# zyc-123/InstanceDiff

Hardware: AMD Instinct MI355X
Metric: denoising steps/sec (256x256 bs16) (higher is better)
Workload: dtype f32; 1 GPU; 256x256 1-ch synthetic, 1000-step reverse chain, batch 16 per GPU, 2 UNet fwd + reverse update per step; global_batch=16, parallelism=replicas x1 (no collective)

## Files before the change

instancediff_amd/csrc/conv_wino4.hip:

```cpp
#include <stdlib.h>

#include <type_traits>

#include "conv_args.h"

using idiff_detail::ConvArgs;

namespace {

constexpr int CK = 4;
constexpr int TW = 32, TH = 16;
constexpr int RCOLS = TW + 2;
constexpr int RS = 40;
constexpr int TRH = TH + 2;
constexpr int PS = TRH * RS;
constexpr int PSP = 768;
constexpr int NT = 512;
constexpr int NL = 6;
constexpr int R_FLOATS = NL * NT;
constexpr int V_FLOATS = 9 * 2 * 64 * 4;
constexpr int U_FLOATS = 9 * 4 * 64 * 4;

typedef float floatx2 __attribute__((ext_vector_type(2)));

__host__ __device__ constexpr int PF(int u) { return (3 * u + 1) / 2; }
__host__ __device__ constexpr int PH(int u) { return 1 + 3 * (u / 2); }
__host__ __device__ constexpr int pos(int u, int v) { return v < 4 ? 4 * PF(u) + v : 4 * PH(u) + 2 * (u & 1) + (v - 4); }

struct Geo4 {
    int np;
    int total;
    int tiles_y8;
};

template <int CTRL>
__device__ __forceinline__ float dpp_row_shr(float v) {
    return __builtin_bit_cast(float, __builtin_amdgcn_update_dpp(0, __builtin_bit_cast(int, v), CTRL, 0xf, 0xf, true));
}
__device__ __forceinline__ float row_sum16(float v) {
    v += dpp_row_shr<0x111>(v);
    v += dpp_row_shr<0x112>(v);
    v += dpp_row_shr<0x114>(v);
    v += dpp_row_shr<0x118>(v);
    return v;
}

#ifdef IDIFF_WINO_TRACE
#define TRACE_PARAM , long long* trace
#define TRACE_INIT long long tr_t[9] = {0, 0, 0, 0, 0, 0, 0, 0, 0}, tr_acc[8] = {0, 0, 0, 0, 0, 0, 0, 0};
#define TRACE_MARK(k)                                                  \
    tr_t[k] = __builtin_readcyclecounter();                            \
    if (k > 0) tr_acc[k - 1] += tr_t[k] - tr_t[k - 1];                 \
    else if (tr_t[3] != 0) tr_acc[3] += tr_t[0] - tr_t[3];
#define TRACE_FINI                                                                                                      \
    if (tid == 0) {                                                                                                     \
        for (int q_ = 0; q_ < 8; ++q_) atomicAdd((unsigned long long*)trace + q_, (unsigned long long)tr_acc[q_]);      \
    }
#else
#define TRACE_PARAM
#define TRACE_INIT
#define TRACE_MARK(k)
#define TRACE_FINI
#endif
#ifdef IDIFF_WINO_SLOTS
#define SLOT_INIT long long sl_acc[10] = {0, 0, 0, 0, 0, 0, 0, 0, 0, 0}, sl_t = 0;
#define SLOT_START sl_t = __builtin_readcyclecounter();
#define SLOT_MARK(k)                                        \
    {                                                       \
        const long long t_ = __builtin_readcyclecounter();  \
        sl_acc[k] += t_ - sl_t;                             \
        sl_t = t_;                                          \
    }
#define SLOT_FINI                                                                                                                   \
    if (lane == 0) {                                                                                                                \
        long long w_ = 0;                                                                                                           \
        for (int q_ = 0; q_ < 9; ++q_) w_ += sl_acc[q_];                                                                            \
        atomicAdd((unsigned long long*)trace + 8 + 2 * wave, (unsigned long long)w_);                                               \
        atomicAdd((unsigned long long*)trace + 9 + 2 * wave, (unsigned long long)sl_acc[9]);                                        \
    }
#else
#define SLOT_INIT
#define SLOT_START
#define SLOT_MARK(k)
#define SLOT_FINI
#endif

__device__ __forceinline__ const float* scalar_ptr(const float* p) {
    const unsigned long long v = reinterpret_cast<unsigned long long>(p);
    const unsigned lo = __builtin_amdgcn_readfirstlane((unsigned)v), hi = __builtin_amdgcn_readfirstlane((unsigned)(v >> 32));
    return reinterpret_cast<const float*>(((unsigned long long)hi << 32) | lo);
}

__device__ __forceinline__ void bt6(const float (&x)[6], float (&o)[6]) {
    o[0] = __builtin_fmaf(4.f, x[0], __builtin_fmaf(-5.f, x[2], x[4]));
    const float p = __builtin_fmaf(-4.f, x[2], x[4]), q = __builtin_fmaf(-4.f, x[1], x[3]);
    o[1] = p + q;
    o[2] = p - q;
    const float c = x[4] - x[2], e = x[3] - x[1];
    o[3] = __builtin_fmaf(2.f, e, c);
    o[4] = __builtin_fmaf(-2.f, e, c);
    o[5] = __builtin_fmaf(4.f, x[1], __builtin_fmaf(-5.f, x[3], x[5]));
}
__device__ __forceinline__ void at6(const float x0, const float x1, const float x2, const float x3, const float x4, const float x5, float (&o)[4]) {
    const float s1 = x1 + x2, d1 = x1 - x2, s2 = x3 + x4, d2 = x3 - x4;
    o[0] = (x0 + s1) + s2;
    o[1] = __builtin_fmaf(2.f, d2, d1);
    o[2] = __builtin_fmaf(4.f, s2, s1);
    o[3] = __builtin_fmaf(8.f, d2, d1) + x5;
}

template <int MODE, int SPEC, bool RAG, bool HEAVY>
__device__ __forceinline__ void conv_wino4_body(const ConvArgs& a, const Geo4& g, float* smem TRACE_PARAM) {
    float* const Rb = smem;
    float* const Vb = smem + 3 * R_FLOATS;
    float* const Ub = Vb + 2 * V_FLOATS;
    float* const econst = Ub + 2 * U_FLOATS;
    int* const gtab = reinterpret_cast<int*>(econst + 512);
    constexpr unsigned R_BYTES = R_FLOATS * 4, U_BYTES = U_FLOATS * 4;
    const unsigned lds_base = __builtin_amdgcn_readfirstlane((unsigned)reinterpret_cast<unsigned long long>(smem));
    const unsigned U_LDS0 = lds_base + (3 * R_FLOATS + 2 * V_FLOATS) * 4;

    const int tid = threadIdx.x;
    const int lane = tid & 63;
    const int wave = __builtin_amdgcn_readfirstlane(tid >> 6);
    const int k4 = lane >> 4;
    const int cb = wave & 3;
    const int tblk = wave >> 2;
    const int HWin = a.Hin * a.Win;
    const int nchunks = a.Cin / CK;

    constexpr int RSRC_FLAGS = 0x00020000;
    struct View {
        int b, co0, y0, x0;
    };
    const float *p0A = a.src0, *p1A = a.src0, *puA = a.wwino4, *p0B = a.src0, *p1B = a.src0, *puB = a.wwino4;
    View vA = {0, 0, 0, 0}, vB = {0, 0, 0, 0};
    int nrB = 0;
    unsigned omaskA = 0, omaskB = 0;
    int it_b = 0, it_cob = 0, it_px = 0, it_py = 0;
    const int tiles_y = g.np / a.tiles_x;
    int d_cob, d_px, d_py, d_b;
    {
        const int G0 = gridDim.x;
        d_cob = G0 % a.ncob;
        const int r1 = G0 / a.ncob;
        d_px = r1 % a.tiles_x;
        const int r2 = r1 / a.tiles_x;
        d_py = r2 % tiles_y;
        d_b = r2 / tiles_y;
    }
    auto decode_first = [&](int item) {
        it_cob = item % a.ncob;
        const int r1 = item / a.ncob;
        it_px = r1 % a.tiles_x;
        const int r2 = r1 / a.tiles_x;
        it_py = r2 % tiles_y;
        it_b = r2 / tiles_y;
    };
    auto advance_item = [&]() {
        it_cob += d_cob;
        int carry = it_cob >= a.ncob;
        it_cob -= carry ? a.ncob : 0;
        it_px += d_px + carry;
        carry = it_px >= a.tiles_x;
        it_px -= carry ? a.tiles_x : 0;
        it_py += d_py + carry;
        carry = it_py >= tiles_y;
        it_py -= carry ? tiles_y : 0;
        it_b += d_b + carry;
    };
    auto decode_B = [&]() {
        vB.b = it_b, vB.co0 = it_cob * 64, vB.y0 = it_py * TH, vB.x0 = it_px * TW;
        puB = scalar_ptr(a.wwino4 + (long long)it_cob * U_FLOATS);
        p0B = scalar_ptr(a.src0 + (long long)it_b * a.bs0);
        p1B = scalar_ptr(SPEC == 3 ? a.src1 + (long long)it_b * a.bs1 : a.src0);
        nrB = 0x7fffffff;
    };
    auto write_table = [&](const View& v) {
        int t = tid;
        asm volatile("" : "+v"(t));
        unsigned om = 0;
#pragma unroll
        for (int i = 0; i < NL; ++i) {
            const int e = t + i * NT;
            const int ci = e / PSP;
            const int rem = e - ci * PSP;
            const int r = rem / RS;
            const int c = rem - r * RS;
            const int oy = v.y0 - 1 + r, ox = v.x0 - 1 + c;
            const bool in = rem < PS && c < RCOLS && (unsigned)oy < (unsigned)a.Hout && (unsigned)ox < (unsigned)a.Wout;
            const int sp = MODE == IDIFF_CONV_UPSAMPLE2 ? (oy >> 1) * a.Win + (ox >> 1) : oy * a.Win + ox;
            gtab[i * NT + tid] = in ? (ci * HWin + sp) * 4 : -1;
            om |= (in ? 0u : 1u) << i;
        }
        return om;
    };
    auto shift_B_to_A = [&]() { p0A = p0B, p1A = p1B, puA = puB, vA = vB, omaskA = omaskB; };
    const int ustride_b = a.ncob * U_FLOATS * 4;

    typedef const __attribute__((address_space(4))) floatx4* cfloatx4p;
    struct Pro {
        floatx4 a, b;
    };
    auto load_pro = [&](int p) {
        Pro r;
        if (SPEC == 2) {
            const bool inA = p < nchunks;
            const long long o = (long long)(inA ? vA.b : vB.b) * a.C0r + (inA ? p : p - nchunks) * CK;
            r.a = *(cfloatx4p)(a.pro_a + o);
            r.b = *(cfloatx4p)(a.pro_b + o);
        }
        return r;
    };

    const unsigned u_voff = tid * 16;
    auto dma_u = [&](int p, int buf) {
        const bool inA = p < nchunks;
        const int so = (inA ? p : p - nchunks) * ustride_b;
        const __amdgpu_buffer_rsrc_t rsu = __builtin_amdgcn_make_buffer_rsrc(const_cast<float*>(inA ? puA : puB), 0, inA ? 0x7fffffff : nrB, RSRC_FLAGS);
        const unsigned lds0 = __builtin_amdgcn_readfirstlane(U_LDS0 + (unsigned)buf * U_BYTES + (unsigned)wave * 1024u);
        asm volatile(
            "s_nop 4\n\ts_mov_b32 m0, %2\n\ts_nop 0\n\tbuffer_load_dwordx4 %0, %1, %3 offen lds\n\t"
            "s_add_u32 m0, m0, 0x2000\n\ts_nop 0\n\tbuffer_load_dwordx4 %0, %1, %4 offen lds\n\t"
            "s_add_u32 m0, m0, 0x2000\n\ts_nop 0\n\tbuffer_load_dwordx4 %0, %1, %5 offen lds\n\t"
            "s_add_u32 m0, m0, 0x2000\n\ts_nop 0\n\tbuffer_load_dwordx4 %0, %1, %6 offen lds"
            ::"v"(u_voff), "s"(rsu), "s"(lds0), "s"(so), "s"(so + NT * 16), "s"(so + 2 * NT * 16), "s"(so + 3 * NT * 16)
            : "memory", "scc");
        if (!HEAVY) {
            const unsigned lds4 = __builtin_amdgcn_readfirstlane(lds0 + 4 * NT * 16 - 256 * 16);
            asm volatile("s_nop 4\n\ts_mov_b32 m0, %2\n\ts_nop 0\n\tbuffer_load_dwordx4 %0, %1, %3 offen lds" ::"v"(u_voff), "s"(rsu), "s"(lds4),
                         "s"(so + 4 * NT * 16 - 256 * 16)
                         : "memory");
        }
    };
    auto dma_u_piece = [&](int p, int buf, int i) {
        const bool inA = p < nchunks;
        const int so = (inA ? p : p - nchunks) * ustride_b + (i < 4 ? i * NT * 16 : 4 * NT * 16 - 256 * 16);
        const __amdgpu_buffer_rsrc_t rsu = __builtin_amdgcn_make_buffer_rsrc(const_cast<float*>(inA ? puA : puB), 0, inA ? 0x7fffffff : nrB, RSRC_FLAGS);
        const unsigned lds0 = __builtin_amdgcn_readfirstlane(U_LDS0 + (unsigned)buf * U_BYTES + (unsigned)wave * 1024u + (unsigned)(i < 4 ? i * NT * 16 : 4 * NT * 16 - 256 * 16));
        asm volatile("s_nop 4\n\ts_mov_b32 m0, %2\n\ts_nop 0\n\tbuffer_load_dwordx4 %0, %1, %3 offen lds" ::"v"(u_voff), "s"(rsu), "s"(lds0), "s"(so) : "memory");
    };
    auto dma_raw = [&](int p, unsigned rslot) {
        const bool inA = p < nchunks;
        const int cbase = (inA ? p : p - nchunks) * CK;
        int goff[NL];
#pragma unroll
        for (int i = 0; i < NL; ++i) goff[i] = gtab[i * NT + tid];
        const int C0v = a.C0v;
        const bool second = SPEC == 3 && cbase >= C0v;
        const unsigned long long b0 = reinterpret_cast<unsigned long long>(inA ? p0A : p0B), b1 = reinterpret_cast<unsigned long long>(inA ? p1A : p1B);
        const float* const base = reinterpret_cast<const float*>(second ? b1 : b0);
        const int so = (second ? cbase - C0v : cbase) * HWin * 4;
        const __amdgpu_buffer_rsrc_t rs = __builtin_amdgcn_make_buffer_rsrc(const_cast<float*>(base), 0, inA ? 0x7fffffff : nrB, RSRC_FLAGS);
        const unsigned lds0 = __builtin_amdgcn_readfirstlane(lds_base + rslot + (unsigned)wave * 256u);
        asm volatile(
            "s_nop 4\n\ts_mov_b32 m0, %8\n\ts_nop 0\n\tbuffer_load_dword %0, %6, %7 offen lds\n\t"
            "s_add_u32 m0, m0, 0x800\n\ts_nop 0\n\tbuffer_load_dword %1, %6, %7 offen lds\n\t"
            "s_add_u32 m0, m0, 0x800\n\ts_nop 0\n\tbuffer_load_dword %2, %6, %7 offen lds\n\t"
            "s_add_u32 m0, m0, 0x800\n\ts_nop 0\n\tbuffer_load_dword %3, %6, %7 offen lds\n\t"
            "s_add_u32 m0, m0, 0x800\n\ts_nop 0\n\tbuffer_load_dword %4, %6, %7 offen lds\n\t"
            "s_add_u32 m0, m0, 0x800\n\ts_nop 0\n\tbuffer_load_dword %5, %6, %7 offen lds"
            ::"v"(goff[0]), "v"(goff[1]), "v"(goff[2]), "v"(goff[3]), "v"(goff[4]), "v"(goff[5]), "s"(rs), "s"(so), "s"(lds0)
            : "memory", "scc");
    };
    auto dma_raw_piece = [&](int p, unsigned rslot, int i, int goff_i) {
        const bool inA = p < nchunks;
        const int cbase = (inA ? p : p - nchunks) * CK;
        const int C0v = a.C0v;
        const bool second = SPEC == 3 && cbase >= C0v;
        const unsigned long long b0 = reinterpret_cast<unsigned long long>(inA ? p0A : p0B), b1 = reinterpret_cast<unsigned long long>(inA ? p1A : p1B);
        const float* const base = reinterpret_cast<const float*>(second ? b1 : b0);
        const int so = (second ? cbase - C0v : cbase) * HWin * 4;
        const __amdgpu_buffer_rsrc_t rs = __builtin_amdgcn_make_buffer_rsrc(const_cast<float*>(base), 0, inA ? 0x7fffffff : nrB, RSRC_FLAGS);
        const unsigned lds0 = __builtin_amdgcn_readfirstlane(lds_base + rslot + (unsigned)wave * 256u + (unsigned)i * 2048u);
        asm volatile("s_nop 4\n\ts_mov_b32 m0, %3\n\ts_nop 0\n\tbuffer_load_dword %0, %1, %2 offen lds" ::"v"(goff_i), "s"(rs), "s"(so), "s"(lds0) : "memory");
    };
    float rinA[NL], rinB[NL];
    auto ld_raw = [&](float (&dst)[NL], int p, int i, int goff_i) {
        const bool inA = p < nchunks;
        const int so = (inA ? p : p - nchunks) * CK * HWin * 4;
        const __amdgpu_buffer_rsrc_t rs = __builtin_amdgcn_make_buffer_rsrc(const_cast<float*>(inA ? p0A : p0B), 0, inA ? 0x7fffffff : nrB, RSRC_FLAGS);
        asm volatile("s_nop 4\n\tbuffer_load_dword %0, %1, %2, %3 offen" : "=v"(dst[i]) : "v"(goff_i), "s"(rs), "s"(so) : "memory");
    };
    auto stage_act = [&](const float (&src)[NL], int p, const Pro& pro, unsigned rslot, int i0, int i1) {
        const unsigned om = p < nchunks ? omaskA : omaskB;
        float* const R = reinterpret_cast<float*>(reinterpret_cast<char*>(Rb) + rslot) + tid;
        constexpr bool hiw = !HEAVY;
#pragma unroll
        for (int i = 0; i < NL; ++i) {
            if (i < i0 || i >= i1) continue;
            const float pa = i == 0 ? pro.a.x : i == 1 ? (hiw ? pro.a.y : pro.a.x) : i == 2 ? pro.a.y : i == 3 ? pro.a.z : i == 4 ? (hiw ? pro.a.w : pro.a.z) : pro.a.w;
            const float pb = i == 0 ? pro.b.x : i == 1 ? (hiw ? pro.b.y : pro.b.x) : i == 2 ? pro.b.y : i == 3 ? pro.b.z : i == 4 ? (hiw ? pro.b.w : pro.b.z) : pro.b.w;
            const float x = silu_fast(pa * src[i] + pb);
            R[i * NT] = ((om >> i) & 1u) ? 0.f : x;
        }
    };
    constexpr int N_U = HEAVY ? 4 : 5;

    constexpr bool heavy = HEAVY;
    const int trole = wave & 1;
    const int thalf = (wave >> 1) & 1;
    const int tx = lane & 7, tyl = (lane >> 3) & 1;
    const float al = trole ? -1.f : -4.f, be = trole ? 2.f : 1.f;
    const float* const trbase = Rb + k4 * PSP + (4 * (2 * thalf + tyl) + (heavy ? 1 : trole)) * RS + 4 * tx;
    const int ufirst = heavy ? 1 + 2 * trole : 5 * trole;
    float* const vwbase = Vb + thalf * 256 + lane * 4;
    float ta[6], tb[6], tlo[6], thi[6];
    auto rd_row = [&](const float* p, float (&d)[6]) {
        const floatx4 lo = *reinterpret_cast<const floatx4*>(p);
        const floatx2 hi = *reinterpret_cast<const floatx2*>(p + 4);
        d[0] = lo.x, d[1] = lo.y, d[2] = lo.z, d[3] = lo.w, d[4] = hi.x, d[5] = hi.y;
    };
    auto tr_piece = [&](int piece, unsigned rslot, int buf) {
        const float* p = reinterpret_cast<const float*>(reinterpret_cast<const char*>(trbase) + rslot);
        if (piece == 0) {
            if (heavy) rd_row(p + 1 * RS, ta), rd_row(p + 3 * RS, tb);
            else rd_row(p, ta), rd_row(p + 2 * RS, tb);
        } else if (piece == 1) {
            if (heavy) {
#pragma unroll
                for (int c = 0; c < 6; ++c) tlo[c] = __builtin_fmaf(al, ta[c], tb[c]);
                rd_row(p, ta), rd_row(p + 2 * RS, tb);
            } else {
#pragma unroll
                for (int c = 0; c < 6; ++c) tlo[c] = __builtin_fmaf(4.f, ta[c], -5.f * tb[c]);
                rd_row(p + 4 * RS, ta);
            }
        } else if (piece == 2) {
            if (heavy) {
#pragma unroll
                for (int c = 0; c < 6; ++c) {
                    const float X = tlo[c], Y = __builtin_fmaf(al, ta[c], tb[c]);
                    tlo[c] = __builtin_fmaf(be, Y, X);
                    thi[c] = __builtin_fmaf(-be, Y, X);
                }
            } else {
#pragma unroll
                for (int c = 0; c < 6; ++c) tlo[c] += ta[c];
            }
        } else {
            const int which = piece - 3;
            if (which == 1 && !heavy) return;
            float o[6];
            bt6(which ? thi : tlo, o);
            const int u = ufirst + which;
            float* const V = vwbase + buf * V_FLOATS;
            *reinterpret_cast<floatx4*>(V + PF(u) * 512) = floatx4{o[0], o[1], o[2], o[3]};
            *reinterpret_cast<floatx2*>(V + PH(u) * 512 + 2 * (u & 1)) = floatx2{o[4], o[5]};
        }
    };

    const int G = gridDim.x;
    const int first = (int)xcd_remap(blockIdx.x, G);
    const int last = g.total;
    if (first >= last) return;
    auto fetch_consts = [&](const View& v) {
        float e = 0.f;
        if (HEAVY) {
            const int which = tid >> 6, co = v.co0 + (tid & 63);
            if (co < a.Cout) {
                if (which == 0 && a.bias) e = a.bias[co];
                if (which == 1 && a.vec) e = a.vec[(long long)v.b * a.Cout + co];
                if (which == 2 && a.aux) e = a.aux_a[(long long)v.b * a.Cout + co];
                if (which == 3 && a.aux) e = a.aux_b[(long long)v.b * a.Cout + co];
            }
        }
        return e;
    };
    TRACE_INIT
    SLOT_INIT

    decode_first(first);
    decode_B();
    shift_B_to_A();
    omaskA = write_table(vA);
    if (first + G < last) {
        advance_item();
        decode_B();
    } else {
        nrB = 0, vB = vA;
    }
    {
        const float e0 = fetch_consts(vA);
        if (HEAVY) econst[tid] = e0;
    }
    dma_u(0, 0);
    if (SPEC != 2) {
        dma_raw(0, 0 * R_BYTES);
        dma_raw(1, 1 * R_BYTES);
        dma_raw(2, 2 * R_BYTES);
        asm volatile("s_waitcnt vmcnt(%0)" ::"n"(NL) : "memory");
        __syncthreads();
    } else {
        int goff[NL];
#pragma unroll
        for (int i = 0; i < NL; ++i) goff[i] = gtab[i * NT + tid];
#pragma unroll
        for (int i = 0; i < NL; ++i) ld_raw(rinA, 0, i, goff[i]);
#pragma unroll
        for (int i = 0; i < NL; ++i) ld_raw(rinB, 1, i, goff[i]);
        const Pro pro0 = load_pro(0), pro1 = load_pro(1);
        asm volatile("s_waitcnt vmcnt(0)" : "+v"(rinA[0]), "+v"(rinA[1]), "+v"(rinA[2]), "+v"(rinA[3]), "+v"(rinA[4]), "+v"(rinA[5]), "+v"(rinB[0]),
                     "+v"(rinB[1]), "+v"(rinB[2]), "+v"(rinB[3]), "+v"(rinB[4]), "+v"(rinB[5])::"memory");
        stage_act(rinA, 0, pro0, 0 * R_BYTES, 0, NL);
        stage_act(rinB, 1, pro1, 1 * R_BYTES, 0, NL);
#pragma unroll
        for (int i = 0; i < NL; ++i) ld_raw(rinA, 2, i, goff[i]);
        __syncthreads();
    }
#pragma unroll
    for (int piece = 0; piece < 5; ++piece) tr_piece(piece, 0 * R_BYTES, 0);
    if (SPEC == 2) asm volatile("s_waitcnt vmcnt(0)" : "+v"(rinA[0]), "+v"(rinA[1]), "+v"(rinA[2]), "+v"(rinA[3]), "+v"(rinA[4]), "+v"(rinA[5])::"memory");
    else asm volatile("s_waitcnt vmcnt(0)" ::: "memory");
    __syncthreads();
    dma_u(1, 1);

    unsigned r_t = 1 * R_BYTES, r_a = 2 * R_BYTES, r_x = 0 * R_BYTES;
    int epar = 0;
    bool young = false;
    for (int item = first; item < last; item += G) {
        TRACE_MARK(0)
        floatx4 acc[36];
        {
            const int opoff = lane * 4;
            floatx4 ob[2], oa[2];
            ob[0] = *reinterpret_cast<const floatx4*>(Vb + tblk * 256 + opoff);
            oa[0] = *reinterpret_cast<const floatx4*>(Ub + cb * 256 + opoff);
            auto chunk = [&](int cc, auto par_tag, auto zero_tag) {
                constexpr int PAR = decltype(par_tag)::value;
                constexpr bool ZERO = decltype(zero_tag)::value;
                const float* V = Vb + PAR * V_FLOATS + tblk * 256 + opoff;
                const float* U = Ub + PAR * U_FLOATS + cb * 256 + opoff;
                const float* Vn = Vb + (PAR ^ 1) * V_FLOATS + tblk * 256 + opoff;
                const float* Un = Ub + (PAR ^ 1) * U_FLOATS + cb * 256 + opoff;
                int goff[NL];
                if (cc + 3 == nchunks) omaskB = write_table(vB);
#pragma unroll
                for (int i = 0; i < NL; ++i) goff[i] = gtab[i * NT + tid];
                float(&rin_s)[NL] = PAR ? rinB : rinA;
                float(&rin_l)[NL] = PAR ? rinA : rinB;
                Pro pro;
                if (SPEC == 2) pro = load_pro(cc + 2);
                SLOT_START
#pragma unroll
                for (int q = 0; q < 9; ++q) {
                    if (q + 1 < 9) {
                        ob[(q + 1 + PAR) & 1] = *reinterpret_cast<const floatx4*>(V + (q + 1) * 512);
                        oa[(q + 1 + PAR) & 1] = *reinterpret_cast<const floatx4*>(U + (q + 1) * 1024);
                    } else {
                        if (young) asm volatile("s_waitcnt vmcnt(%0)" ::"n"(NL + (RAG ? 0 : 16)) : "memory");
                        else asm volatile("s_waitcnt vmcnt(%0)" ::"n"(NL) : "memory");
                        young = false;
                        __builtin_amdgcn_sched_barrier(0);
                        SLOT_MARK(8)
                        __syncthreads();
                        SLOT_MARK(9)
                        if (cc + 1 == nchunks) dma_u(cc + 2, PAR);
                        else dma_u_piece(cc + 2, PAR, 0);
                        ob[PAR ^ 1] = *reinterpret_cast<const floatx4*>(Vn);
                        oa[PAR ^ 1] = *reinterpret_cast<const floatx4*>(Un);
                    }
                    const floatx4 bv = ob[(q + PAR) & 1], av = oa[(q + PAR) & 1];
                    const floatx4 z4 = floatx4{0.f, 0.f, 0.f, 0.f};
                    acc[4 * q + 0] = __builtin_amdgcn_mfma_f32_16x16x4f32(av.x, bv.x, ZERO ? z4 : acc[4 * q + 0], 0, 0, 0);
                    acc[4 * q + 1] = __builtin_amdgcn_mfma_f32_16x16x4f32(av.y, bv.y, ZERO ? z4 : acc[4 * q + 1], 0, 0, 0);
                    acc[4 * q + 2] = __builtin_amdgcn_mfma_f32_16x16x4f32(av.z, bv.z, ZERO ? z4 : acc[4 * q + 2], 0, 0, 0);
                    acc[4 * q + 3] = __builtin_amdgcn_mfma_f32_16x16x4f32(av.w, bv.w, ZERO ? z4 : acc[4 * q + 3], 0, 0, 0);
                    if (!ZERO) {
                        if (q < 3) dma_u_piece(cc + 1, PAR ^ 1, q + 1);
                        if (q == 3 && !HEAVY) dma_u_piece(cc + 1, PAR ^ 1, 4);
                    }
                    if (SPEC == 2 && q == 5) {
                        if (young) asm volatile("s_waitcnt vmcnt(%6)" : "+v"(rin_s[0]), "+v"(rin_s[1]), "+v"(rin_s[2]), "+v"(rin_s[3]), "+v"(rin_s[4]), "+v"(rin_s[5]) : "n"(N_U + 2 + (RAG ? 0 : 16)) : "memory");
                        else asm volatile("s_waitcnt vmcnt(%6)" : "+v"(rin_s[0]), "+v"(rin_s[1]), "+v"(rin_s[2]), "+v"(rin_s[3]), "+v"(rin_s[4]), "+v"(rin_s[5]) : "n"(N_U + 2) : "memory");
                        stage_act(rin_s, cc + 2, pro, r_a, 0, 2);
                    }
                    if (SPEC == 2 && q == 6) stage_act(rin_s, cc + 2, pro, r_a, 2, 4);
                    if (SPEC == 2 && q == 7) stage_act(rin_s, cc + 2, pro, r_a, 4, 6);
                    auto req = [&](int i) {
                        if (SPEC == 2) ld_raw(rin_l, cc + 3, i, goff[i]);
                        else dma_raw_piece(cc + 3, r_x, i, goff[i]);
                    };
                    if (HEAVY && q == 3) req(0);
                    if (!HEAVY && q == 4) req(0);
                    if (q == 4) req(1);
                    if (q == 5) req(2);
                    if (q == 6) req(3);
                    if (q == 7) req(4), req(5);
                    if (q < 5) tr_piece(q, r_t, PAR ^ 1);
                    __builtin_amdgcn_sched_barrier(0);
                    if (q < 8) { SLOT_MARK(q) }
                }
                const unsigned t = r_t;
                r_t = r_a, r_a = r_x, r_x = t;
            };
            chunk(0, std::integral_constant<int, 0>{}, std::true_type{});
            chunk(1, std::integral_constant<int, 1>{}, std::false_type{});
            for (int cc = 2; cc < nchunks; cc += 2) {
                chunk(cc, std::integral_constant<int, 0>{}, std::false_type{});
                chunk(cc + 1, std::integral_constant<int, 1>{}, std::false_type{});
            }
        }
        TRACE_MARK(1)

        const View v = vA;
        const float* const ebase_item = econst + epar * 256;
        const bool more = item + G < last;
        float pre_e = 0.f;
        if (more) {
            shift_B_to_A();
            if (item + 2 * G < last) {
                advance_item();
                decode_B();
            } else {
                nrB = 0, vB = vA;
            }
            pre_e = fetch_consts(vA);
        }
        young = true;

        const int b = v.b, co0 = v.co0, y0 = v.y0, x0 = v.x0;
        {
            int lane_e = lane;
            asm volatile("" : "+v"(lane_e));
            const int j = lane_e & 15, k4 = lane_e >> 4;
            const int HWo = a.Hout * a.Wout;
            const int ty0 = y0 + 8 * tblk;
            const bool wave_live = co0 + cb * 16 < a.Cout;
            const long long wave_org = (long long)(co0 + cb * 16) * HWo + (long long)ty0 * a.Wout + x0;
            const __amdgpu_buffer_rsrc_t rso = __builtin_amdgcn_make_buffer_rsrc(const_cast<float*>(scalar_ptr(a.out + (long long)b * a.obs + wave_org)), 0, wave_live ? 0x7fffffff : 0, RSRC_FLAGS);
            const float* const resb = a.res ? a.res + (long long)b * a.rbs + wave_org : nullptr;
            const float* const auxb = a.aux ? a.aux + (long long)b * a.abs_ + wave_org : nullptr;
            const bool inside = !RAG || ((ty0 + 4 * (j >> 3) < a.Hout) && (x0 + 4 * (j & 7) < a.Wout));
            const unsigned lane_off = (unsigned)(4 * k4) * (unsigned)HWo + (unsigned)(4 * (j >> 3)) * (unsigned)a.Wout + 4u * (j & 7);
            const float* const ebase = ebase_item + cb * 16 + 4 * k4;
            const bool want_stats = a.stats != nullptr && ty0 < a.Hout && wave_live;
            const bool has_res = a.res != nullptr && wave_live, has_aux = a.aux != nullptr && wave_live;
            const float* const stbase = a.stats ? a.stats + (((long long)b * a.ntiles + (ty0 >> 3) * a.tiles_x + (x0 >> 5)) * a.Cout + co0 + cb * 16) * 2 : a.out;
            const __amdgpu_buffer_rsrc_t rst = __builtin_amdgcn_make_buffer_rsrc(const_cast<float*>(scalar_ptr(stbase)), 0, want_stats ? 0x7fffffff : 0, RSRC_FLAGS);
            constexpr int AUX_SC1 = 1 << 4;
            float zz[6][4][4];
#pragma unroll
            for (int u = 0; u < 6; ++u) {
#pragma unroll
                for (int r = 0; r < 4; ++r) {
                    at6(acc[pos(u, 0)][r], acc[pos(u, 1)][r], acc[pos(u, 2)][r], acc[pos(u, 3)][r], acc[pos(u, 4)][r], acc[pos(u, 5)][r], zz[u][r]);
                    asm volatile("" : "+v"(zz[u][r][0]), "+v"(zz[u][r][1]), "+v"(zz[u][r][2]), "+v"(zz[u][r][3]));
                }
                __builtin_amdgcn_sched_barrier(0);
            }
            TRACE_MARK(2)
            floatx4 nres = floatx4{0.f, 0.f, 0.f, 0.f}, naux = nres;
#ifdef W4_STATS_LAST
            typedef unsigned uintx2_ __attribute__((ext_vector_type(2)));
            uintx2_ spr[4];
#endif
            auto fetch = [&](int s) {
                if (!inside) return;
                const long long so = (long long)(s >> 2) * HWo + (s & 3) * a.Wout;
                if (has_res) nres = *reinterpret_cast<const floatx4*>(resb + so + lane_off);
                if (has_aux) naux = *reinterpret_cast<const floatx4*>(auxb + so + lane_off);
            };
            fetch(0);
#pragma unroll
            for (int r = 0; r < 4; ++r) {
                const float bv = ebase[r];
                float y[4][4];
#pragma unroll
                for (int x = 0; x < 4; ++x) {
                    float col[4];
                    at6(zz[0][r][x], zz[1][r][x], zz[2][r][x], zz[3][r][x], zz[4][r][x], zz[5][r][x], col);
#pragma unroll
                    for (int dy = 0; dy < 4; ++dy) y[dy][x] = col[dy] + bv;
                }
                {
                    float ssum = 0.f, ssq = 0.f;
                    if (a.stats != nullptr) {
#pragma unroll
                        for (int dy = 0; dy < 4; ++dy) {
                            ssum += (y[dy][0] + y[dy][1]) + (y[dy][2] + y[dy][3]);
                            ssq += (y[dy][0] * y[dy][0] + y[dy][1] * y[dy][1]) + (y[dy][2] * y[dy][2] + y[dy][3] * y[dy][3]);
                        }
                        if (!inside) ssum = 0.f, ssq = 0.f;
                        ssum = row_sum16(ssum);
                        ssq = row_sum16(ssq);
                    }
                    typedef unsigned uintx2 __attribute__((ext_vector_type(2)));
                    const uintx2 pr = {__builtin_bit_cast(unsigned, ssum), __builtin_bit_cast(unsigned, ssq)};
#ifndef W4_STATS_LAST
                    __builtin_amdgcn_raw_buffer_store_b64(pr, rst, j == 15 ? (4 * k4 + r) * 8 : -1, 0, AUX_SC1);
#else
                    spr[r] = pr;
#endif
                }
                const float add = ebase[64 + r];
                float aa = 0.f, ab = 0.f;
                if (has_aux) aa = ebase[128 + r], ab = ebase[192 + r];
#pragma unroll
                for (int dy = 0; dy < 4; ++dy) {
                    const floatx4 cres = nres, caux = naux;
                    if (4 * r + dy + 1 < 16) fetch(4 * r + dy + 1);
                    floatx4 v4 = floatx4{y[dy][0] + add, y[dy][1] + add, y[dy][2] + add, y[dy][3] + add};
                    if (has_res) v4 += cres;
                    if (has_aux) {
                        v4.x += silu_fast(aa * caux.x + ab), v4.y += silu_fast(aa * caux.y + ab);
                        v4.z += silu_fast(aa * caux.z + ab), v4.w += silu_fast(aa * caux.w + ab);
                    }
                    typedef unsigned uintx4 __attribute__((ext_vector_type(4)));
                    if (!RAG || inside) __builtin_amdgcn_raw_buffer_store_b128(__builtin_bit_cast(uintx4, v4), rso, (int)(lane_off * 4u), (r * HWo + dy * a.Wout) * 4, 0);
                }
                __builtin_amdgcn_sched_barrier(0);
            }
#ifdef W4_STATS_LAST
#pragma unroll
            for (int r = 0; r < 4; ++r) __builtin_amdgcn_raw_buffer_store_b64(spr[r], rst, j == 15 ? (4 * k4 + r) * 8 : -1, 0, AUX_SC1);
#endif
        }
        TRACE_MARK(3)
        if (HEAVY && more) econst[(epar ^ 1) * 256 + tid] = pre_e;
        epar ^= 1;
    }
    asm volatile("s_waitcnt vmcnt(0)" ::: "memory");
    TRACE_FINI
    SLOT_FINI
}

template <int MODE, int SPEC, bool RAG>
__global__ __launch_bounds__(NT) void conv_wino4_kernel(const ConvArgs a, const Geo4 g TRACE_PARAM) {
    extern __shared__ __attribute__((aligned(16))) float smem[];
#ifdef IDIFF_WINO_TRACE
    if (__builtin_amdgcn_readfirstlane(threadIdx.x >> 6) < 4) conv_wino4_body<MODE, SPEC, RAG, true>(a, g, smem, trace);
    else conv_wino4_body<MODE, SPEC, RAG, false>(a, g, smem, trace);
#else
    if (__builtin_amdgcn_readfirstlane(threadIdx.x >> 6) < 4) conv_wino4_body<MODE, SPEC, RAG, true>(a, g, smem);
    else conv_wino4_body<MODE, SPEC, RAG, false>(a, g, smem);
#endif
}

template <int MODE, int SPEC, bool RAG>
int launch_rag(const ConvArgs& a, hipStream_t st) {
    const size_t lds = ((size_t)3 * R_FLOATS + 2 * V_FLOATS + 2 * U_FLOATS + 2 * 256 + NL * NT) * sizeof(float);
    if (lds > 160 * 1024) IDIFF_FAIL(IDIFF_E_UNSUPPORTED, "conv2d(winograd4): LDS budget exceeded (%zu bytes)", lds);
    static idiff_dyn_lds_cache lds_cache;
    auto kern = conv_wino4_kernel<MODE, SPEC, RAG>;
    {
        hipError_t e = idiff_ensure_dyn_lds(lds_cache, reinterpret_cast<const void*>(kern), lds);
        if (e != hipSuccess) IDIFF_FAIL(IDIFF_E_HIP, "conv2d(winograd4): hipFuncSetAttribute: %s", hipGetErrorString(e));
    }
    static int num_cu = 0;
    if (num_cu == 0) {
        int dev = 0, n = 0;
        if (hipGetDevice(&dev) != hipSuccess || hipDeviceGetAttribute(&n, hipDeviceAttributeMultiprocessorCount, dev) != hipSuccess || n <= 0)
            IDIFF_FAIL(IDIFF_E_HIP, "conv2d(winograd4): cannot query the CU count");
        num_cu = n;
    }
    Geo4 g;
    const int tiles_y16 = (a.Hout + TH - 1) / TH;
    g.np = a.tiles_x * tiles_y16;
    g.tiles_y8 = (a.Hout + 7) / 8;
    const long long total = (long long)a.B * g.np * a.ncob;
    if (total >= (1ll << 31)) IDIFF_FAIL(IDIFF_E_BADARG, "conv2d(winograd4): grid too large");
    g.total = (int)total;
    const int per = (g.total + num_cu - 1) / num_cu;
    const int grid = (g.total + per - 1) / per;
#ifdef IDIFF_WINO_TRACE
    static long long* tr = nullptr;
    if (!tr) (void)hipMalloc(&tr, 32 * sizeof(long long));
    (void)hipMemsetAsync(tr, 0, 32 * sizeof(long long), st);
    hipLaunchKernelGGL(kern, dim3(grid), dim3(NT), lds, st, a, g, tr);
    long long h[32];
    (void)hipMemcpyAsync(h, tr, sizeof(h), hipMemcpyDeviceToHost, st);
    (void)hipStreamSynchronize(st);
    fprintf(stderr, "[wino4 trace] Cin=%d Cout=%d H=%d items=%d per=%d | main loop %lld | switch + output transform %lld | statistics + stores %lld | to next item %lld (cycles/item, wave 0)\n",
            a.Cin, a.Cout, a.Hout, g.total, per, h[0] / g.total, h[1] / g.total, h[2] / g.total, h[3] / g.total);
#ifdef IDIFF_WINO_SLOTS
    {
        const long long nch = (long long)g.total * (a.Cin / CK - 1);
        fprintf(stderr, "[wino4 slots] Cin=%d H=%d work/barrier-wait cycles per chunk, waves 0..7:", a.Cin, a.Hout);
        for (int w = 0; w < 8; ++w) fprintf(stderr, " %lld/%lld", h[8 + 2 * w] / nch, h[9 + 2 * w] / nch);
        fprintf(stderr, "\n");
    }
#endif
#else
    hipLaunchKernelGGL(kern, dim3(grid), dim3(NT), lds, st, a, g);
#endif
    IDIFF_CHECK_LAUNCH("conv2d_fwd(winograd4)");
    return IDIFF_OK;
}

template <int MODE, int SPEC>
int launch(const ConvArgs& a, hipStream_t st) {
    if (a.Hout % TH || a.Wout % TW) return launch_rag<MODE, SPEC, true>(a, st);
    return launch_rag<MODE, SPEC, false>(a, st);
}

__global__ void pack_wino4_kernel(const float* __restrict__ w, float* __restrict__ out, int Cout, int Cin, int transpose) {
    const int Co = transpose ? Cin : Cout, Ci = transpose ? Cout : Cin;
    const int ncob = (Co + 63) / 64;
    const long long n = (long long)Co * Ci;
    for (long long i = blockIdx.x * (long long)blockDim.x + threadIdx.x; i < n; i += (long long)gridDim.x * blockDim.x) {
        const int co = i % Co, ci = i / Co;
        float gk[3][3];
#pragma unroll
        for (int p = 0; p < 3; ++p)
#pragma unroll
            for (int q = 0; q < 3; ++q)
                gk[p][q] = transpose ? w[((long long)ci * Cin + co) * 9 + (2 - p) * 3 + (2 - q)] : w[((long long)co * Cin + ci) * 9 + p * 3 + q];
        auto g6 = [](float x0, float x1, float x2, float(&o)[6]) {
            o[0] = 0.25f * x0;
            const float s = x0 + x2;
            o[1] = (-1.f / 6.f) * (s + x1);
            o[2] = (-1.f / 6.f) * (s - x1);
            const float t = __builtin_fmaf(4.f, x2, x0);
            o[3] = (1.f / 24.f) * __builtin_fmaf(2.f, x1, t);
            o[4] = (1.f / 24.f) * __builtin_fmaf(-2.f, x1, t);
            o[5] = x2;
        };
        float t[6][3];
#pragma unroll
        for (int q = 0; q < 3; ++q) {
            float o[6];
            g6(gk[0][q], gk[1][q], gk[2][q], o);
#pragma unroll
            for (int u = 0; u < 6; ++u) t[u][q] = o[u];
        }
        const int cc = ci >> 2, kk = ci & 3;
        const int cbk = co >> 6, col = co & 63, cb = col >> 4, i16 = col & 15;
        float* dst = out + ((long long)cc * ncob + cbk) * U_FLOATS + cb * 256 + (kk * 16 + i16) * 4;
#pragma unroll
        for (int u = 0; u < 6; ++u) {
            float o[6];
            g6(t[u][0], t[u][1], t[u][2], o);
#pragma unroll
            for (int v = 0; v < 6; ++v) {
                const int p = pos(u, v);
                dst[(p >> 2) * 1024 + (p & 3)] = o[v];
            }
        }
    }
}

int wino4_mode() {
    static const int m = [] {
        const char* e = getenv("IDIFF_WINOGRAD4");
        return e ? atoi(e) : 1;
    }();
    return m;
}
}

namespace idiff_detail {

long long conv_wino4_items(const ConvArgs& a, int ks, int mode, bool requested) {
    if (ks != 3 || !a.wwino4 || (wino4_mode() == 0 && !requested)) return 0;
    if (mode != IDIFF_CONV_NORMAL && mode != IDIFF_CONV_UPSAMPLE2) return 0;
    if (a.Cout % 16 || a.Cin % 8 || a.C0v % CK || (a.Hout & 3) || (a.Wout & 3) || a.Wout < 24) return 0;
    if ((long long)a.Cin * a.Hin * a.Win * 4 >= (1ll << 31)) return 0;
    if (144ll * a.Cin * a.ncob * 64 + U_FLOATS * 4 >= (1ll << 31)) return 0;
    if (mode == IDIFF_CONV_UPSAMPLE2 && (a.pro_a || a.src1)) return 0;
    if (a.pro_a && a.src1) return 0;
    if (a.pro_a && ((a.C0r & 3) || (reinterpret_cast<uintptr_t>(a.pro_a) & 15) || (reinterpret_cast<uintptr_t>(a.pro_b) & 15))) return 0;
    if ((reinterpret_cast<uintptr_t>(a.wwino4) & 15) != 0) return 0;
    if ((a.obs & 3) || (a.res && (a.rbs & 3)) || (a.aux && (a.abs_ & 3))) return 0;
    if ((reinterpret_cast<uintptr_t>(a.out) & 15) || (reinterpret_cast<uintptr_t>(a.res) & 15) || (reinterpret_cast<uintptr_t>(a.aux) & 15)) return 0;
    return (long long)a.tiles_x * ((a.Hout + TH - 1) / TH) * a.ncob;
}

int launch_conv_wino4(const ConvArgs& a, int mode, hipStream_t st) {
#ifdef W4_ONLY
    return launch_rag<IDIFF_CONV_NORMAL, 1, false>(a, st);
#else
    if (mode == IDIFF_CONV_UPSAMPLE2) return launch<IDIFF_CONV_UPSAMPLE2, 1>(a, st);
    if (a.pro_a) return launch<IDIFF_CONV_NORMAL, 2>(a, st);
    if (a.src1) return launch<IDIFF_CONV_NORMAL, 3>(a, st);
    return launch<IDIFF_CONV_NORMAL, 1>(a, st);
#endif
}

}

extern "C" int idiff_pack_conv_weight_wino4(const float* w, float* wwino4, int Cout, int Cin, int transpose, idiff_stream_t stream) {
    IDIFF_CHECK_ARG(w && wwino4 && Cout > 0 && Cin > 0, "pack_conv_weight_wino4: bad args");
    const int Co = transpose ? Cin : Cout, Ci = transpose ? Cout : Cin;
    IDIFF_CHECK_ARG(Co % 16 == 0 && Ci % 8 == 0, "pack_conv_weight_wino4: needs conv Cout %% 16 == 0 and Cin %% 8 == 0 (got %d, %d)", Co, Ci);
    if (Co % 64) {
        hipError_t e = hipMemsetAsync(wwino4, 0, (size_t)36 * Ci * ((Co + 63) / 64) * 64 * sizeof(float), (hipStream_t)stream);
        if (e != hipSuccess) IDIFF_FAIL(IDIFF_E_HIP, "pack_conv_weight_wino4: hipMemsetAsync: %s", hipGetErrorString(e));
    }
    const long long n = (long long)Cout * Cin;
    const int grid = (int)((n + 255) / 256 > 4096 ? 4096 : (n + 255) / 256);
    hipLaunchKernelGGL(pack_wino4_kernel, dim3(grid), dim3(256), 0, (hipStream_t)stream, w, wwino4, Cout, Cin, transpose);
    IDIFF_CHECK_LAUNCH("pack_conv_weight_wino4");
    return IDIFF_OK;
}
```

Measured before the change: 43.84 steps/s.

## Remap SPEC 2 activation staging to five dense load rounds per thread

For the SPEC 2 path (activation prologue applied in registers), each thread now loads five elements instead of six. Each wave pair covers half of a channel's padded halo tile with a dense row/column map, and a precomputed LDS address table scatters the results into the strided layout. Idle lanes write into the channel's unused tail region. This cuts one global load, one SiLU evaluation and some wasted padded-slot traffic per chunk, and trims the vmcnt waits to match. An optional packed two-wide SiLU path sits behind a macro that is off by default.

Result: no change. 44.01 steps/s, median of 6 (+0.4%).

```diff
diff --git a/instancediff_amd/csrc/conv_wino4.hip b/instancediff_amd/csrc/conv_wino4.hip
--- a/instancediff_amd/csrc/conv_wino4.hip
+++ b/instancediff_amd/csrc/conv_wino4.hip
@@ -18,10 +18,16 @@
 constexpr int NT = 512;
 constexpr int NL = 6;
 constexpr int R_FLOATS = NL * NT;
+constexpr int NA = 5;
+constexpr int AH = TRH * RCOLS / 2;
+static_assert(NA * 64 >= AH && (NA - 1) * 64 < AH && NA * 64 - AH <= PSP - PS, "SPEC 2 staging map: five rounds, the idle lanes' dump fits the channel's tail");
 constexpr int V_FLOATS = 9 * 2 * 64 * 4;
 constexpr int U_FLOATS = 9 * 4 * 64 * 4;
 
 typedef float floatx2 __attribute__((ext_vector_type(2)));
+#ifndef W4_PRO_PACKED
+#define W4_PRO_PACKED 0
+#endif
 
 __host__ __device__ constexpr int PF(int u) { return (3 * u + 1) / 2; }
 __host__ __device__ constexpr int PH(int u) { return 1 + 3 * (u / 2); }
@@ -180,6 +186,18 @@
         int t = tid;
         asm volatile("" : "+v"(t));
         unsigned om = 0;
+        if (SPEC == 2) {
+#pragma unroll
+            for (int i = 0; i < NA; ++i) {
+                const int k = (t & 63) + 64 * i, e = (wave & 1) * AH + k;
+                const int r = e / RCOLS, c = e - r * RCOLS;
+                const int oy = v.y0 - 1 + r, ox = v.x0 - 1 + c;
+                const bool in = k < AH && (unsigned)oy < (unsigned)a.Hout && (unsigned)ox < (unsigned)a.Wout;
+                gtab[i * NT + tid] = in ? ((wave >> 1) * HWin + oy * a.Win + ox) * 4 : -1;
+                om |= (in ? 1u : 0u) << i;
+            }
+            return om;
+        }
 #pragma unroll
         for (int i = 0; i < NL; ++i) {
             const int e = t + i * NT;
@@ -275,27 +293,50 @@
         const unsigned lds0 = __builtin_amdgcn_readfirstlane(lds_base + rslot + (unsigned)wave * 256u + (unsigned)i * 2048u);
         asm volatile("s_nop 4\n\ts_mov_b32 m0, %3\n\ts_nop 0\n\tbuffer_load_dword %0, %1, %2 offen lds" ::"v"(goff_i), "s"(rs), "s"(so), "s"(lds0) : "memory");
     };
-    float rinA[NL], rinB[NL];
-    auto ld_raw = [&](float (&dst)[NL], int p, int i, int goff_i) {
+    float rinA[NA], rinB[NA];
+    auto ld_raw = [&](float (&dst)[NA], int p, int i, int goff_i) {
         const bool inA = p < nchunks;
         const int so = (inA ? p : p - nchunks) * CK * HWin * 4;
         const __amdgpu_buffer_rsrc_t rs = __builtin_amdgcn_make_buffer_rsrc(const_cast<float*>(inA ? p0A : p0B), 0, inA ? 0x7fffffff : nrB, RSRC_FLAGS);
         asm volatile("s_nop 4\n\tbuffer_load_dword %0, %1, %2, %3 offen" : "=v"(dst[i]) : "v"(goff_i), "s"(rs), "s"(so) : "memory");
     };
-    auto stage_act = [&](const float (&src)[NL], int p, const Pro& pro, unsigned rslot, int i0, int i1) {
+    unsigned radr[NA];
+    if (SPEC == 2) {
+#pragma unroll
+        for (int i = 0; i < NA; ++i) {
+            const int k = lane + 64 * i, e = (wave & 1) * AH + k;
+            const int r = e / RCOLS, c = e - r * RCOLS;
+            radr[i] = (unsigned)((wave >> 1) * PSP + (k < AH ? r * RS + c : PS + (k - AH))) * 4u;
+            asm volatile("" : "+v"(radr[i]));
+        }
+    }
+    auto stage_act = [&](const float (&src)[NA], int p, const Pro& pro, unsigned rslot, int i0, int i1) {
         const unsigned om = p < nchunks ? omaskA : omaskB;
-        float* const R = reinterpret_cast<float*>(reinterpret_cast<char*>(Rb) + rslot) + tid;
-        constexpr bool hiw = !HEAVY;
-#pragma unroll
-        for (int i = 0; i < NL; ++i) {
-            if (i < i0 || i >= i1) continue;
-            const float pa = i == 0 ? pro.a.x : i == 1 ? (hiw ? pro.a.y : pro.a.x) : i == 2 ? pro.a.y : i == 3 ? pro.a.z : i == 4 ? (hiw ? pro.a.w : pro.a.z) : pro.a.w;
-            const float pb = i == 0 ? pro.b.x : i == 1 ? (hiw ? pro.b.y : pro.b.x) : i == 2 ? pro.b.y : i == 3 ? pro.b.z : i == 4 ? (hiw ? pro.b.w : pro.b.z) : pro.b.w;
-            const float x = silu_fast(pa * src[i] + pb);
-            R[i * NT] = ((om >> i) & 1u) ? 0.f : x;
+        char* const R = reinterpret_cast<char*>(Rb) + rslot;
+        const bool odd = (wave & 2) != 0;
+        const float pa = HEAVY ? (odd ? pro.a.y : pro.a.x) : (odd ? pro.a.w : pro.a.z);
+        const float pb = HEAVY ? (odd ? pro.b.y : pro.b.x) : (odd ? pro.b.w : pro.b.z);
+        constexpr float NLOG2E = -0x1.715476p+0f;
+        auto put = [&](int i, float x) {
+            const int keep = (int)(om << (31 - i)) >> 31;
+            *reinterpret_cast<int*>(R + radr[i]) = __builtin_bit_cast(int, x) & keep;
+        };
+        if (W4_PRO_PACKED && i1 - i0 == 2) {
+            const floatx2 v = __builtin_elementwise_fma(floatx2{pa, pa}, floatx2{src[i0], src[i0 + 1]}, floatx2{pb, pb});
+            const floatx2 t = v * floatx2{NLOG2E, NLOG2E};
+            const floatx2 d = floatx2{1.0f, 1.0f} + floatx2{__builtin_amdgcn_exp2f(t.x), __builtin_amdgcn_exp2f(t.y)};
+            const floatx2 x = v * floatx2{__builtin_amdgcn_rcpf(d.x), __builtin_amdgcn_rcpf(d.y)};
+            put(i0, x.x), put(i0 + 1, x.y);
+        } else {
+#pragma unroll
+            for (int i = 0; i < NA; ++i) {
+                if (i < i0 || i >= i1) continue;
+                put(i, silu_fast(pa * src[i] + pb));
+            }
         }
     };
     constexpr int N_U = HEAVY ? 4 : 5;
+    constexpr int NRQ = SPEC == 2 ? NA : NL;
 
     constexpr bool heavy = HEAVY;
     const int trole = wave & 1;
@@ -392,25 +433,25 @@
         asm volatile("s_waitcnt vmcnt(%0)" ::"n"(NL) : "memory");
         __syncthreads();
     } else {
-        int goff[NL];
-#pragma unroll
-        for (int i = 0; i < NL; ++i) goff[i] = gtab[i * NT + tid];
-#pragma unroll
-        for (int i = 0; i < NL; ++i) ld_raw(rinA, 0, i, goff[i]);
-#pragma unroll
-        for (int i = 0; i < NL; ++i) ld_raw(rinB, 1, i, goff[i]);
+        int goff[NA];
+#pragma unroll
+        for (int i = 0; i < NA; ++i) goff[i] = gtab[i * NT + tid];
+#pragma unroll
+        for (int i = 0; i < NA; ++i) ld_raw(rinA, 0, i, goff[i]);
+#pragma unroll
+        for (int i = 0; i < NA; ++i) ld_raw(rinB, 1, i, goff[i]);
         const Pro pro0 = load_pro(0), pro1 = load_pro(1);
-        asm volatile("s_waitcnt vmcnt(0)" : "+v"(rinA[0]), "+v"(rinA[1]), "+v"(rinA[2]), "+v"(rinA[3]), "+v"(rinA[4]), "+v"(rinA[5]), "+v"(rinB[0]),
-                     "+v"(rinB[1]), "+v"(rinB[2]), "+v"(rinB[3]), "+v"(rinB[4]), "+v"(rinB[5])::"memory");
-        stage_act(rinA, 0, pro0, 0 * R_BYTES, 0, NL);
-        stage_act(rinB, 1, pro1, 1 * R_BYTES, 0, NL);
-#pragma unroll
-        for (int i = 0; i < NL; ++i) ld_raw(rinA, 2, i, goff[i]);
+        asm volatile("s_waitcnt vmcnt(0)" : "+v"(rinA[0]), "+v"(rinA[1]), "+v"(rinA[2]), "+v"(rinA[3]), "+v"(rinA[4]), "+v"(rinB[0]),
+                     "+v"(rinB[1]), "+v"(rinB[2]), "+v"(rinB[3]), "+v"(rinB[4])::"memory");
+        stage_act(rinA, 0, pro0, 0 * R_BYTES, 0, 2), stage_act(rinA, 0, pro0, 0 * R_BYTES, 2, 4), stage_act(rinA, 0, pro0, 0 * R_BYTES, 4, 5);
+        stage_act(rinB, 1, pro1, 1 * R_BYTES, 0, 2), stage_act(rinB, 1, pro1, 1 * R_BYTES, 2, 4), stage_act(rinB, 1, pro1, 1 * R_BYTES, 4, 5);
+#pragma unroll
+        for (int i = 0; i < NA; ++i) ld_raw(rinA, 2, i, goff[i]);
         __syncthreads();
     }
 #pragma unroll
     for (int piece = 0; piece < 5; ++piece) tr_piece(piece, 0 * R_BYTES, 0);
-    if (SPEC == 2) asm volatile("s_waitcnt vmcnt(0)" : "+v"(rinA[0]), "+v"(rinA[1]), "+v"(rinA[2]), "+v"(rinA[3]), "+v"(rinA[4]), "+v"(rinA[5])::"memory");
+    if (SPEC == 2) asm volatile("s_waitcnt vmcnt(0)" : "+v"(rinA[0]), "+v"(rinA[1]), "+v"(rinA[2]), "+v"(rinA[3]), "+v"(rinA[4])::"memory");
     else asm volatile("s_waitcnt vmcnt(0)" ::: "memory");
     __syncthreads();
     dma_u(1, 1);
@@ -436,9 +477,9 @@
                 int goff[NL];
                 if (cc + 3 == nchunks) omaskB = write_table(vB);
 #pragma unroll
-                for (int i = 0; i < NL; ++i) goff[i] = gtab[i * NT + tid];
-                float(&rin_s)[NL] = PAR ? rinB : rinA;
-                float(&rin_l)[NL] = PAR ? rinA : rinB;
+                for (int i = 0; i < NRQ; ++i) goff[i] = gtab[i * NT + tid];
+                float(&rin_s)[NA] = PAR ? rinB : rinA;
+                float(&rin_l)[NA] = PAR ? rinA : rinB;
                 Pro pro;
                 if (SPEC == 2) pro = load_pro(cc + 2);
                 SLOT_START
@@ -448,8 +489,8 @@
                         ob[(q + 1 + PAR) & 1] = *reinterpret_cast<const floatx4*>(V + (q + 1) * 512);
                         oa[(q + 1 + PAR) & 1] = *reinterpret_cast<const floatx4*>(U + (q + 1) * 1024);
                     } else {
-                        if (young) asm volatile("s_waitcnt vmcnt(%0)" ::"n"(NL + (RAG ? 0 : 16)) : "memory");
-                        else asm volatile("s_waitcnt vmcnt(%0)" ::"n"(NL) : "memory");
+                        if (young) asm volatile("s_waitcnt vmcnt(%0)" ::"n"(NRQ + (RAG ? 0 : 16)) : "memory");
+                        else asm volatile("s_waitcnt vmcnt(%0)" ::"n"(NRQ) : "memory");
                         young = false;
                         __builtin_amdgcn_sched_barrier(0);
                         SLOT_MARK(8)
@@ -471,14 +512,14 @@
                         if (q == 3 && !HEAVY) dma_u_piece(cc + 1, PAR ^ 1, 4);
                     }
                     if (SPEC == 2 && q == 5) {
-                        if (young) asm volatile("s_waitcnt vmcnt(%6)" : "+v"(rin_s[0]), "+v"(rin_s[1]), "+v"(rin_s[2]), "+v"(rin_s[3]), "+v"(rin_s[4]), "+v"(rin_s[5]) : "n"(N_U + 2 + (RAG ? 0 : 16)) : "memory");
-                        else asm volatile("s_waitcnt vmcnt(%6)" : "+v"(rin_s[0]), "+v"(rin_s[1]), "+v"(rin_s[2]), "+v"(rin_s[3]), "+v"(rin_s[4]), "+v"(rin_s[5]) : "n"(N_U + 2) : "memory");
+                        if (young) asm volatile("s_waitcnt vmcnt(%5)" : "+v"(rin_s[0]), "+v"(rin_s[1]), "+v"(rin_s[2]), "+v"(rin_s[3]), "+v"(rin_s[4]) : "n"(N_U + 2 + (RAG ? 0 : 16)) : "memory");
+                        else asm volatile("s_waitcnt vmcnt(%5)" : "+v"(rin_s[0]), "+v"(rin_s[1]), "+v"(rin_s[2]), "+v"(rin_s[3]), "+v"(rin_s[4]) : "n"(N_U + 2) : "memory");
                         stage_act(rin_s, cc + 2, pro, r_a, 0, 2);
                     }
                     if (SPEC == 2 && q == 6) stage_act(rin_s, cc + 2, pro, r_a, 2, 4);
-                    if (SPEC == 2 && q == 7) stage_act(rin_s, cc + 2, pro, r_a, 4, 6);
+                    if (SPEC == 2 && q == 7) stage_act(rin_s, cc + 2, pro, r_a, 4, 5);
                     auto req = [&](int i) {
-                        if (SPEC == 2) ld_raw(rin_l, cc + 3, i, goff[i]);
+                        if (SPEC == 2) ld_raw(rin_l, cc + 3, i < NA ? i : 0, goff[i]);
                         else dma_raw_piece(cc + 3, r_x, i, goff[i]);
                     };
                     if (HEAVY && q == 3) req(0);
@@ -486,7 +527,8 @@
                     if (q == 4) req(1);
                     if (q == 5) req(2);
                     if (q == 6) req(3);
-                    if (q == 7) req(4), req(5);
+                    if (q == 7) req(4);
+                    if (q == 7 && SPEC != 2) req(5);
                     if (q < 5) tr_piece(q, r_t, PAR ^ 1);
                     __builtin_amdgcn_sched_barrier(0);
                     if (q < 8) { SLOT_MARK(q) }
```
